# cloudflare/circl

Measured on AMD Instinct MI355X. Metric: ML-KEM-768 encapsulations/sec (whole node), batch=2^20, higher is better.
Workload: dtype i32; 1 GPU; ML-KEM-768 Encapsulate, distinct-key (one GPU-generated key per item), batch=1048576 per GPU, inputs resident in HBM (SURVEY 8d scope i; the PCIe-inclusive host-ABI rate, scope ii, is `value_host_abi`); key_pool=1048576, parallelism=batch split per device, no collectives, mode=encaps

## Files before the change

### circl_amd/csrc/api_mlkem.hip

```cpp
#include "host_compose.h"
#include "keytable.h"
#include "mlkem_kernels.h"

#include <type_traits>
#include <utility>

using namespace circl::host;
using circl::KeyIdx;

namespace {

constexpr size_t kKemWsPerItem = 129;
size_t kem_scratch_bytes() { return 256 + max_resident_blocks() * 64 * 512; }
size_t kem_small_batch() {
    static const size_t v = [] {
        const char *e = getenv("CIRCL_HIP_KEM_SMALL");
        const int lg = e ? atoi(e) : 15;
        return lg <= 0 ? size_t(0) : size_t(1) << std::min(lg, 20);
    }();
    return v;
}
size_t kem_coop_batch() {
    static const size_t v = [] {
        const char *e = getenv("CIRCL_HIP_KEM_COOP");
// ... 42 lines not shown
    switch (kem_k(param)) {
    case 2: return f(std::integral_constant<int, 2>{});
    case 3: return f(std::integral_constant<int, 3>{});
    case 4: return f(std::integral_constant<int, 4>{});
    }
    return unknown;
}
template <class F> int kem_dev_call(int param, void *stream, F &&f) {
    if (ndev() <= 0) return CIRCL_HIP_ENODEV;
    hipStream_t st = static_cast<hipStream_t>(stream);
    return kem_with_k(param, [&](auto k) -> int { return f(k, st); });
}

template <int K> struct KemTable {
    uint8_t *base;
    size_t nkeys, padded;
    KemTable(void *b, size_t nk)
        : base(static_cast<uint8_t *>(b)), nkeys(nk), padded((nk + circl::mlkem::Geom<K>::G - 1) / circl::mlkem::Geom<K>::G * circl::mlkem::Geom<K>::G) {}
    size_t rows_bytes() const { return up256(padded * K * K * 512); }
    int16_t *rows() const { return reinterpret_cast<int16_t *>(base); }
    uint8_t *h() const { return base + rows_bytes(); }
    uint8_t *status() const { return h() + up256(nkeys * 32); }
    size_t bytes() const { return rows_bytes() + up256(nkeys * 32) + up256(nkeys); }
};
size_t kem_table_bytes_any(int param, size_t nkeys) {
    return kem_with_k(param, [&](auto k) { return KemTable<k.value>(nullptr, nkeys).bytes(); }, size_t(0));
}

struct KemWs {
    uint8_t *slot0, *slot1, *slot2, *slot3, *status_slot;
    unsigned *work;
    uint8_t *scratch;
    KemWs(void *ws, size_t n) {
        slot0 = static_cast<uint8_t *>(ws);
        slot1 = slot0 + 32 * n;
        slot2 = slot0 + 64 * n;
        slot3 = slot0 + 96 * n;
        status_slot = slot0 + 128 * n;
        work = reinterpret_cast<unsigned *>(slot0 + up256(kKemWsPerItem * n));
        scratch = slot0 + up256(kKemWsPerItem * n) + 256;
    }
};


struct KemEncArgs {
    const uint8_t *ek = nullptr;
    size_t stride = 0;
    const uint8_t *m = nullptr, *r = nullptr;
    uint8_t *ct = nullptr, *ss = nullptr, *status = nullptr;
    KeyIdx kx{};
    const int16_t *key_rows = nullptr;
    const uint8_t *kbar = nullptr, *ssrej = nullptr;
};
template <int K, int MODE, int KM> void kem_encrypt(const KemWs &w, size_t n, size_t want, const KemEncArgs &a, hipStream_t st) {
    using Gm = circl::mlkem::Geom<K>;
    constexpr int lds = KM == circl::mlkem::KM_ITEM ? Gm::LDS_SCRATCH_TOTAL : Gm::LDS_SHARED_TOTAL;
    ProfScope ps(CIRCL_HIP_KERNEL_MLKEM_ENCRYPT, st);
    auto kern = circl::mlkem::mlkem_encrypt_kernel<K, MODE, 0, true, KM>;
    const unsigned eb = std::min<unsigned>((unsigned)((n + want - 1) / want), resident_blocks(kern, lds));
    hipLaunchKernelGGL(kern, dim3(eb), dim3(64), lds, st, a.ek, a.stride, a.m, a.r, a.ct, a.ss, a.status, a.kbar, a.ssrej, w.scratch, w.work, n, a.kx,
                       a.key_rows);
}

template <int K, bool R3 = false>
int encaps_dev_impl(const uint8_t *ek, const uint8_t *m, uint8_t *ct, uint8_t *ss, uint8_t *status, size_t n,
                    void *ws, size_t ws_bytes, hipStream_t st) {
    using Gm = circl::mlkem::Geom<K>;
    using namespace circl::mlkem;
    if (n == 0) return CIRCL_HIP_OK;
    if (ws_bytes < kem_ws_min(n) || !aligned<16>(ws, ek, m, ct, ss))
        return CIRCL_HIP_EWORKSPACE;
    KemWs w(ws, n);
    uint8_t *r_ws = w.slot0, *m_ws = w.slot1;
    const unsigned hb = (unsigned)((n + 255) / 256);
    if (!R3 && n <= kem_chain_item_batch()) {
        ProfScope ps(CIRCL_HIP_KERNEL_MLKEM_ENCRYPT, st);
        hipLaunchKernelGGL((mlkem_encaps_chain_kernel<K, false>), dim3((unsigned)n), dim3(128), 0, st, ek, (size_t)Gm::EK, KeyIdx{},
                           (const int16_t *)nullptr, (const uint8_t *)nullptr, m, ct, ss, status, n);
        HIP_TRY(hipGetLastError());
        return CIRCL_HIP_OK;
    }
    if (!R3 && kem_small_route(n, ws_bytes)) {
        int16_t *key_rows = reinterpret_cast<int16_t *>(static_cast<uint8_t *>(ws) + kem_small_table_ofs(n));
        const int coop = kem_hash_form(n, kem_coop_batch());
        const unsigned nb_expand = (unsigned)((n + Gm::G - 1) / Gm::G), nb_hash = kem_hash_blocks(n, coop);
        static_assert(Gm::LDS_FIFO >= 108 * 8, "the cooperative hash's exchange area fits the FIFO area");
        HIP_TRY(hipMemsetAsync(w.work, 0, 256, st));
        {
            ProfScope ps(CIRCL_HIP_KERNEL_MLKEM_HASH, st);
            hipLaunchKernelGGL(mlkem_small_pre_kernel<K>, dim3(nb_hash + nb_expand), dim3(64), Gm::LDS_FIFO, st, ek, m, ss, r_ws, key_rows, n, nb_hash, coop);
        }
        kem_encrypt<K, ENCAPS, KM_KEYED>(w, n, kem_small_group(n), {ek, (size_t)Gm::EK, m, r_ws, ct, ss, status, KeyIdx{}, key_rows}, st);
        HIP_TRY(hipGetLastError());
        return CIRCL_HIP_OK;
    }
    HIP_TRY(hipMemsetAsync(w.work, 0, 256, st));
    {
        ProfScope ps(CIRCL_HIP_KERNEL_MLKEM_HASH, st);
        if (R3) hipLaunchKernelGGL(kyber_r3_hash_kernel<K>, dim3(hb), dim3(256), 0, st, ek, m, ss, r_ws, m_ws, n);
        else hipLaunchKernelGGL(mlkem_hash_kernel<K>, dim3(hb), dim3(256), 0, st, ek, m, ss, r_ws, n);
    }
    kem_encrypt<K, R3 ? ENCAPS_LENIENT : ENCAPS, KM_ITEM>(w, n, Gm::G, {ek, (size_t)Gm::EK, R3 ? (const uint8_t *)m_ws : m, r_ws, ct, ss, status}, st);
    if (R3) {
        ProfScope ps(CIRCL_HIP_KERNEL_MLKEM_HASH, st);
        hipLaunchKernelGGL(kyber_r3_finish_kernel<K>, dim3(hb), dim3(256), 0, st, (const uint8_t *)ct, ss, n);
    }
    HIP_TRY(hipGetLastError());
    return CIRCL_HIP_OK;
}

template <int K>
int encaps_shared_dev_impl(const uint8_t *ek, const uint8_t *m, uint8_t *ct, uint8_t *ss, uint8_t *status, size_t n, void *ws,
                           size_t ws_bytes, hipStream_t st) {
    using Gm = circl::mlkem::Geom<K>;
    using namespace circl::mlkem;
    if (n == 0) return CIRCL_HIP_OK;
    if (ws_bytes < kem_ws_min(n) || !aligned<16>(ws, ek, m, ct, ss))
        return CIRCL_HIP_EWORKSPACE;
    KemWs w(ws, n);
    uint8_t *r_ws = w.slot0, *h_ws = w.slot1;
    if (n <= kem_chain_item_batch()) {
        ProfScope ps(CIRCL_HIP_KERNEL_MLKEM_ENCRYPT, st);
        hipLaunchKernelGGL((mlkem_encaps_chain_kernel<K, false>), dim3((unsigned)n), dim3(128), 0, st, ek, (size_t)0, KeyIdx{},
                           (const int16_t *)nullptr, (const uint8_t *)nullptr, m, ct, ss, status, n);
        HIP_TRY(hipGetLastError());
        return CIRCL_HIP_OK;
    }
    HIP_TRY(hipMemsetAsync(w.work, 0, 256, st));
    if (n <= kem_small_shared_batch(false)) {
        int16_t *key_rows = reinterpret_cast<int16_t *>(static_cast<uint8_t *>(ws) + kem_small_table_ofs(n));
        static_assert(Gm::LDS_FIFO >= 108 * 8, "the cooperative hash's exchange area fits the FIFO area");
        {
            ProfScope ps(CIRCL_HIP_KERNEL_MLKEM_HASH, st);
            hipLaunchKernelGGL(mlkem_small_shared_pre_kernel<K>, dim3(1 + (unsigned)((n + 31) / 32)), dim3(64), Gm::LDS_FIFO, st, ek, m, ss, r_ws, key_rows, n);
        }
        kem_encrypt<K, ENCAPS, KM_KEYED>(w, n, kem_small_group(n), {ek, 0, m, r_ws, ct, ss, status, KeyIdx{}, key_rows}, st);
        HIP_TRY(hipGetLastError());
        return CIRCL_HIP_OK;
    }
    {
        ProfScope ps(CIRCL_HIP_KERNEL_MLKEM_HASH, st);
        hipLaunchKernelGGL(mlkem_hek_kernel<K>, dim3(1), dim3(64), 0, st, ek, h_ws);
        hipLaunchKernelGGL(mlkem_g_shared_kernel, dim3((unsigned)((n + 255) / 256)), dim3(256), 0, st, (const uint8_t *)h_ws, m, ss,
                           r_ws, n, KeyIdx{});
    }
    kem_encrypt<K, ENCAPS, KM_SHARED>(w, n, Gm::GS, {ek, 0, m, r_ws, ct, ss, status}, st);
    HIP_TRY(hipGetLastError());
    return CIRCL_HIP_OK;
}

template <int K>
int decaps_shared_dev_impl(const uint8_t *dk, const uint8_t *ct, uint8_t *ss, uint8_t *status, size_t n, void *ws, size_t ws_bytes,
                           hipStream_t st) {
    using Gm = circl::mlkem::Geom<K>;
    using namespace circl::mlkem;
// ... 71 lines not shown
                               mprime, kbar, r_ws, ssrej, status, (uint8_t *)nullptr, key_rows, n, nb_hash, nb_hash, coop);
        }
        kem_encrypt<K, REENCRYPT, KM_KEYED>(w, n, kem_small_group(n, true),
                                            {dk + 384 * K, (size_t)Gm::DK, mprime, r_ws, const_cast<uint8_t *>(ct), ss, status, KeyIdx{}, key_rows, kbar, ssrej}, st);
        HIP_TRY(hipGetLastError());
        return CIRCL_HIP_OK;
    }
    {
        ProfScope ps(CIRCL_HIP_KERNEL_MLKEM_DECRYPT, st);
        hipLaunchKernelGGL(mlkem_decrypt_kernel<K>, dim3((unsigned)n), dim3(64), 0, st, dk, (size_t)Gm::DK, ct, mprime, n, KeyIdx{});
    }
    {
        ProfScope ps(CIRCL_HIP_KERNEL_MLKEM_HASH, st);
        if (R3)
            hipLaunchKernelGGL(kyber_r3_decaps_hash_kernel<K>, dim3(hb), dim3(256), 0, st, dk, (const uint8_t *)mprime, kbar, r_ws,
                               ssrej, status, n);
        else
            hipLaunchKernelGGL(mlkem_decaps_hash_kernel<K>, dim3(hb), dim3(256), 0, st, dk, (size_t)Gm::DK, ct, (const uint8_t *)mprime,
                               kbar, r_ws, ssrej, status, n, (const uint8_t *)nullptr, KeyIdx{});
    }
    kem_encrypt<K, REENCRYPT, KM_ITEM>(w, n, Gm::G,
                                       {dk + 384 * K, (size_t)Gm::DK, mprime, r_ws, const_cast<uint8_t *>(ct), ss, status, KeyIdx{}, nullptr, kbar, ssrej}, st);
    if (R3) {
        ProfScope ps(CIRCL_HIP_KERNEL_MLKEM_HASH, st);
        hipLaunchKernelGGL(kyber_r3_finish_kernel<K>, dim3(hb), dim3(256), 0, st, ct, ss, n);
    }
    HIP_TRY(hipGetLastError());
    return CIRCL_HIP_OK;
}

template <int K, bool R3 = false>
int keygen_dev_impl(const uint8_t *seed64, uint8_t *ek, uint8_t *dk, size_t n, void *ws, size_t ws_bytes, hipStream_t st) {
    using Gm = circl::mlkem::Geom<K>;
    using namespace circl::mlkem;
    if (n == 0) return CIRCL_HIP_OK;
    if (ws_bytes < kem_ws_min(n) || !aligned<16>(ws, seed64, ek, dk)) return CIRCL_HIP_EWORKSPACE;
    KemWs w(ws, n);
    uint8_t *rs = w.slot0;
    if (n <= kem_chain_item_batch()) {
        ProfScope ps(CIRCL_HIP_KERNEL_MLKEM_KEYGEN, st);
        hipLaunchKernelGGL((mlkem_keygen_chain_kernel<K, R3>), dim3((unsigned)n), dim3(128), 0, st, seed64, ek, dk, n);
        HIP_TRY(hipGetLastError());
        return CIRCL_HIP_OK;
    }
    HIP_TRY(hipMemsetAsync(w.work, 0, 256, st));
    const unsigned hb = (unsigned)((n + 255) / 256);
    {
        ProfScope ps(CIRCL_HIP_KERNEL_MLKEM_HASH, st);
        hipLaunchKernelGGL((mlkem_keygen_seed_kernel<K, R3>), dim3(hb), dim3(256), 0, st, seed64, rs, n);
    }
    {
        ProfScope ps(CIRCL_HIP_KERNEL_MLKEM_KEYGEN, st);
        auto kern = mlkem_keygen_kernel<K, true>;
        const unsigned kb = std::min<unsigned>((unsigned)((n + Gm::G - 1) / Gm::G), resident_blocks(kern, Gm::LDS_SCRATCH_TOTAL));
        hipLaunchKernelGGL(kern, dim3(kb), dim3(64), Gm::LDS_SCRATCH_TOTAL, st, (const uint8_t *)rs, ek, dk, w.scratch, w.work, n);
    }
    {
        ProfScope ps(CIRCL_HIP_KERNEL_MLKEM_FINISH, st);
        const int form = n <= (size_t(1) << 15) ? kem_hash_form(n, kem_coop_batch()) : 0;
        if (form) hipLaunchKernelGGL(mlkem_keygen_finish_small_kernel<K>, dim3(kem_hash_blocks(n, form)), dim3(64), 0, st, seed64, (const uint8_t *)ek, dk, n, form);
        else hipLaunchKernelGGL(mlkem_keygen_finish_kernel<K>, dim3(hb), dim3(256), 0, st, seed64, (const uint8_t *)ek, dk, n);
    }
    HIP_TRY(hipGetLastError());
    return CIRCL_HIP_OK;
}


template <int K> void kem_table_fill(const KemTable<K> &tb, const uint8_t *keys, size_t row, bool private_keys, hipStream_t st) {
    using Gm = circl::mlkem::Geom<K>;
    using namespace circl::mlkem;
    const size_t ek_off = private_keys ? 384 * K : 0, rho_off = ek_off + 384 * K;
    hipLaunchKernelGGL(mlkem_hek_table_kernel<K>, dim3((unsigned)((tb.nkeys + 255) / 256)), dim3(256), 0, st, keys, row, ek_off, tb.h(),
                       private_keys ? tb.status() : (uint8_t *)nullptr, private_keys ? 1 : 0, tb.nkeys);
    hipLaunchKernelGGL(mlkem_expand_keys_kernel<K>, dim3((unsigned)(tb.padded / Gm::G)), dim3(64), Gm::LDS_FIFO, st, keys, row, rho_off, tb.rows(), tb.nkeys);
}

template <int K>
int encaps_with_table(const KemTable<K> &tb, const uint8_t *keys, size_t stride, KeyIdx kx, bool latency, const uint8_t *m, uint8_t *ct, uint8_t *ss,
                      uint8_t *status, size_t n, const KemWs &w, hipStream_t st) {
    using Gm = circl::mlkem::Geom<K>;
    using namespace circl::mlkem;
    uint8_t *r_ws = w.slot0;
    if (latency && n <= kem_chain_batch(false)) {
        ProfScope ps(CIRCL_HIP_KERNEL_MLKEM_ENCRYPT, st);
        circl::TailFlag tail{nullptr, nullptr, 0};
        take_tail_flag(&tail.flag, &tail.count, &tail.value);
        hipLaunchKernelGGL(mlkem_encaps_chain_kernel<K>, dim3((unsigned)n), dim3(64), 0, st, keys, (size_t)Gm::EK, kx, (const int16_t *)tb.rows(),
                           (const uint8_t *)tb.h(), m, ct, ss, status, n, tail);
        HIP_TRY(hipGetLastError());
        return CIRCL_HIP_OK;
    }
    HIP_TRY(hipMemsetAsync(w.work, 0, 256, st));
    {
        ProfScope ps(CIRCL_HIP_KERNEL_MLKEM_HASH, st);
        hipLaunchKernelGGL(mlkem_g_shared_kernel, dim3((unsigned)((n + 255) / 256)), dim3(256), 0, st, (const uint8_t *)tb.h(), m, ss, r_ws, n, kx);
    }
    const size_t want = latency && n <= kem_small_shared_batch(false) ? kem_small_group(n) : (size_t)Gm::GS;
    kem_encrypt<K, ENCAPS, KM_KEYED>(w, n, want, {keys, stride, m, r_ws, ct, ss, status, kx, tb.rows()}, st);
    HIP_TRY(hipGetLastError());
    return CIRCL_HIP_OK;
}
template <int K>
int decaps_with_table(const KemTable<K> &tb, const uint8_t *dk, size_t stride, KeyIdx kx, bool latency, const uint8_t *ct, uint8_t *ss, uint8_t *status,
                      size_t n, const KemWs &w, hipStream_t st) {
    using Gm = circl::mlkem::Geom<K>;
    using namespace circl::mlkem;
    uint8_t *mprime = w.slot0, *r_ws = w.slot1, *kbar = w.slot2, *ssrej = w.slot3;
// ... 446 lines not shown
```

### circl_amd/csrc/mlkem_kernels.h

```cpp
#pragma once
#include "kyber_dev.h"

#ifndef CIRCL_KEM_RING_PRIO
#define CIRCL_KEM_RING_PRIO 1
#endif
#ifndef CIRCL_KEM_WAVES_PER_EU
#define CIRCL_KEM_WAVES_PER_EU 4
#endif

namespace circl {
namespace mlkem {

using kyber::Q;

template <int K> struct Params;
template <> struct Params<2> { static constexpr int ETA1 = 3, DU = 10, DV = 4; };
template <> struct Params<3> { static constexpr int ETA1 = 2, DU = 10, DV = 4; };
template <> struct Params<4> { static constexpr int ETA1 = 2, DU = 11, DV = 5; };

template <int K> struct Geom {
    using P = Params<K>;
    static constexpr int EK = 384 * K + 32;
    static constexpr int DK = 768 * K + 96;
    static constexpr int CT = 32 * (P::DU * K + P::DV);
    static constexpr int PAIRS = K * K;
    static constexpr int G = 64 / PAIRS;
    static constexpr int A_STREAMS = G * PAIRS;
    static constexpr int NOISE = 2 * K + 1;
    static constexpr int A_STRIDE = 520;
    static constexpr int NOISE_BYTES = 64 * P::ETA1;
    static constexpr int NOISE_STRIDE = NOISE_BYTES + 8;
    static constexpr int LDS_A = A_STREAMS * A_STRIDE;
    static constexpr int HALVES = K == 2 ? 2 : 1;
    static constexpr int GH = G / HALVES;
    static constexpr int LDS_NOISE = GH * NOISE * NOISE_STRIDE;
    static constexpr int LDS_XCH = 1024;
    static constexpr int LDS_TOTAL = LDS_A + LDS_NOISE + LDS_XCH;
    static constexpr int FIFO_STRIDE = 80;
    static constexpr int LDS_FIFO = 64 * FIFO_STRIDE;
    static constexpr int LDS_SCRATCH_TOTAL = (LDS_FIFO > LDS_NOISE + LDS_XCH) ? LDS_FIFO : LDS_NOISE + LDS_XCH;
    static constexpr int SCRATCH_BYTES = 64 * 512;
    static constexpr int GS = K == 2 ? 8 : 64 / NOISE;
    static constexpr int LDS_NOISE_SHARED = GS * NOISE * NOISE_STRIDE;
    static constexpr int LDS_SHARED_TOTAL = (LDS_FIFO > LDS_NOISE_SHARED + LDS_XCH) ? LDS_FIFO : LDS_NOISE_SHARED + LDS_XCH;
};


template <int FIRST, int COUNT> __device__ __forceinline__ void xor_words(KeccakState &s, const uint64_t *p) {
    detail::static_for<0, COUNT>([&](auto ic) {
        constexpr int i = decltype(ic)::v;
        const uint64_t w = p[i];
        s.lo[FIRST + i] ^= (uint32_t)w;
        s.hi[FIRST + i] ^= (uint32_t)(w >> 32);
    });
}

template <int NWORDS> __device__ __forceinline__ void sha3_256_words(KeccakState &s, const uint64_t *p) {
    constexpr int FULL = NWORDS / 17, REM = NWORDS % 17;
    keccak_zero(s);
#pragma unroll 1
    for (int b = 0; b < FULL; b++) {
        xor_words<0, 17>(s, p + 17 * b);
        keccak_f1600(s);
    }
    xor_words<0, REM>(s, p + 17 * FULL);
    s.lo[REM] ^= kDsSha3;
    s.hi[16] ^= 0x80000000u;
    keccak_f1600(s);
}

__device__ __forceinline__ void sha3_512_m_h(KeccakState &g, const uint64_t *m, const KeccakState &h) {
    keccak_zero(g);
    xor_words<0, 4>(g, m);
#pragma unroll
    for (int i = 0; i < 4; i++) { g.lo[4 + i] = h.lo[i]; g.hi[4 + i] = h.hi[i]; }
    g.lo[8] = kDsSha3;
    g.hi[8] = 0x80000000u;
    keccak_f1600(g);
}

template <int NWORDS, class Src> __device__ __forceinline__ void split_sponge17_src(SplitState &s, Src &&src, uint32_t ds, bool hi_lane) {
    constexpr int FULL = NWORDS / 17, REM = NWORDS % 17;
    uint32_t nx[17];
#pragma unroll
    for (int j = 0; j < 25; j++) s.w[j] = 0;
#pragma unroll
    for (int j = 0; j < 17; j++) nx[j] = (FULL > 0 || j < REM) ? src(j) : 0;
#pragma unroll 1
    for (int b = 0; b < FULL; b++) {
#pragma unroll
        for (int j = 0; j < 17; j++) s.w[j] ^= nx[j];
        const bool last = b + 1 == FULL;
#pragma unroll
// ... 15 lines not shown
    const uint32_t *mw = reinterpret_cast<const uint32_t *>(m + item * 32) + parity;
    SplitState s;
#pragma unroll
    for (int j = 0; j < 4; j++) { s.w[j] = mw[2 * j]; s.w[4 + j] = h[j]; }
    s.w[8] = hi_lane ? 0x80000000u : kDsSha3;
#pragma unroll
    for (int j = 9; j < 25; j++) s.w[j] = 0;
    keccak_f1600_split(s, hi_lane);
    if (live) {
        uint32_t *kd = reinterpret_cast<uint32_t *>(ss + item * 32) + parity, *rd = reinterpret_cast<uint32_t *>(r_ws + item * 32) + parity;
#pragma unroll
        for (int j = 0; j < 4; j++) { kd[2 * j] = s.w[j]; rd[2 * j] = s.w[4 + j]; }
    }
}
template <int K>
__device__ __forceinline__ void mlkem_hash_split(const uint8_t *__restrict__ ek, const uint8_t *__restrict__ m, uint8_t *__restrict__ ss,
                                                 uint8_t *__restrict__ r_ws, size_t item, bool live, int parity) {
    using Gm = Geom<K>;
    SplitState s;
    split_sponge17<Gm::EK / 8>(s, reinterpret_cast<const uint32_t *>(ek + item * Gm::EK) + parity, kDsSha3, parity != 0);
    const uint32_t h[4] = {s.w[0], s.w[1], s.w[2], s.w[3]};
    mlkem_g_split(h, m, ss, r_ws, item, live, parity);
}

template <int FIRST, int COUNT> __device__ __forceinline__ void store_words(uint64_t *p, const KeccakState &s) {
    detail::static_for<0, COUNT>([&](auto ic) {
        constexpr int i = decltype(ic)::v;
        p[i] = ((uint64_t)s.hi[FIRST + i] << 32) | s.lo[FIRST + i];
    });
}

template <bool NW = false, class Src>
__device__ __forceinline__ void coop_sponge17(uint32_t &vlo, uint32_t &vhi, Src &&src, int nwords, uint32_t ds, const CoopLane &c, int j) {
    const int full = nwords / 17, rem = nwords % 17;
    vlo = vhi = 0;
    uint64_t next = j < 17 ? src(j) : 0;
#pragma unroll 1
    for (int b = 0; b < full; b++) {
        vlo ^= (uint32_t)next;
        vhi ^= (uint32_t)(next >> 32);
        next = (j < 17 && 17 * (b + 1) + j < nwords) ? src(17 * (b + 1) + j) : 0;
        keccak_f1600_coop2<NW>(vlo, vhi, c);
    }
    vlo ^= (uint32_t)next;
    vhi ^= (uint32_t)(next >> 32);
    if (j == rem) vlo ^= ds;
    if (j == 16) vhi ^= 0x80000000u;
    keccak_f1600_coop2<NW>(vlo, vhi, c);
}


template <int K>
__global__ void __launch_bounds__(256) mlkem_hash_kernel(const uint8_t *__restrict__ ek, const uint8_t *__restrict__ m,
                                                         uint8_t *__restrict__ ss, uint8_t *__restrict__ r_ws, size_t n) {
    using Gm = Geom<K>;
    size_t idx = (size_t)blockIdx.x * 256 + threadIdx.x;
    const bool live = idx < n;
    if (!live) idx = n - 1;
    KeccakState h, g;
    sha3_256_words<Gm::EK / 8>(h, reinterpret_cast<const uint64_t *>(ek + idx * Gm::EK));
    sha3_512_m_h(g, reinterpret_cast<const uint64_t *>(m + idx * 32), h);
    if (live) {
        store_words<0, 4>(reinterpret_cast<uint64_t *>(ss + idx * 32), g);
        store_words<4, 4>(reinterpret_cast<uint64_t *>(r_ws + idx * 32), g);
    }
}

template <int K>
__global__ void __launch_bounds__(64) mlkem_dk_check_kernel(const uint8_t *__restrict__ dk, uint8_t *__restrict__ key_status) {
    __shared__ uint64_t ws[100];
    const int lane = threadIdx.x, j = lane & 31;
    const CoopLane c = coop_lane(ws, lane);
    const uint64_t *ekw = reinterpret_cast<const uint64_t *>(dk + 384 * K);
    const uint64_t *stored = reinterpret_cast<const uint64_t *>(dk + 768 * K + 32);
    uint32_t vlo, vhi;
    coop_sponge17(vlo, vhi, [&](int k) { return ekw[k]; }, Geom<K>::EK / 8, kDsSha3, c, j);
    const bool mine = j >= 4 || ((((uint64_t)vhi << 32) | vlo) == stored[j & 3]);
    const unsigned long long bad = __ballot(!mine);
    if (lane == 0) *key_status = (bad & 0xfull) == 0 ? 0 : 2;
}


template <int K>
__global__ void __launch_bounds__(64) mlkem_hek_kernel(const uint8_t *__restrict__ ek, uint8_t *__restrict__ h_ws) {
    __shared__ uint64_t ws[100];
    const int lane = threadIdx.x, j = lane & 31;
    const CoopLane c = coop_lane(ws, lane);
    const uint64_t *ekw = reinterpret_cast<const uint64_t *>(ek);
    uint32_t vlo, vhi;
    coop_sponge17(vlo, vhi, [&](int k) { return ekw[k]; }, Geom<K>::EK / 8, kDsSha3, c, j);
    if (lane < 4) reinterpret_cast<uint64_t *>(h_ws)[lane] = ((uint64_t)vhi << 32) | vlo;
}

template <int K>
__global__ void __launch_bounds__(256) mlkem_hek_table_kernel(const uint8_t *__restrict__ keys, size_t stride, size_t ek_off,
                                                              uint8_t *__restrict__ h_out, uint8_t *__restrict__ key_status, int stored,
                                                              size_t nkeys) {
    size_t j = (size_t)blockIdx.x * 256 + threadIdx.x;
    const bool live = j < nkeys;
    if (!live) j = nkeys - 1;
    const uint8_t *ekp = keys + j * stride + ek_off;
    KeccakState h;
    sha3_256_words<Geom<K>::EK / 8>(h, reinterpret_cast<const uint64_t *>(ekp));
    if (!live) return;
    store_words<0, 4>(reinterpret_cast<uint64_t *>(h_out + j * 32), h);
    if (stored) {
        const uint64_t *st = reinterpret_cast<const uint64_t *>(ekp + Geom<K>::EK);
        bool ok = true;
#pragma unroll
        for (int i = 0; i < 4; i++) ok &= (((uint64_t)h.hi[i] << 32) | h.lo[i]) == st[i];
        key_status[j] = ok ? 0 : 2;
    }
}
// ... 142 lines not shown
            fifo[cnt & (SLOTS - 1)] = (int16_t)v;
            count_accept(cnt, v);
            if constexpr (c % 8 == 7) {
                cnt = min(cnt, 256);
                if (cnt - flushed >= 8) {
                    const uint4 d = *reinterpret_cast<const uint4 *>(fifo + (flushed & (SLOTS - 1)));
                    *reinterpret_cast<uint4 *>(row + flushed) = d;
                    flushed += 8;
                }
                if constexpr (TAIL) live = __any(flushed < 256);
            }
        }
    });
}

template <int K, bool TRANSPOSED, int GA = Geom<K>::G, bool XY_ARG = false>
__device__ __forceinline__ void sample_matrix_scratch(uint8_t *lds_fifo, int16_t *rows, const uint8_t *__restrict__ rho,
                                                      size_t rho_stride, size_t item0, size_t n, int lane, const uint8_t *__restrict__ xy = nullptr) {
    using Gm = Geom<K>;
    const bool on = XY_ARG ? item0 + lane < n : lane < GA * Gm::PAIRS;
    const int g = XY_ARG ? lane : on ? lane / Gm::PAIRS : 0, p = on ? lane % Gm::PAIRS : 0;
    const int i = p / K, j = p % K;
    size_t item = item0 + g;
    if (item >= n) item = n - 1;
    KeccakState s;
    keccak_zero(s);
    xor_words<0, 4>(s, reinterpret_cast<const uint64_t *>(rho + item * rho_stride));
    if constexpr (XY_ARG) s.lo[4] = (uint32_t)xy[2 * item] | ((uint32_t)xy[2 * item + 1] << 8) | (kDsShake << 16);
    else s.lo[4] = (TRANSPOSED ? (uint32_t)i | ((uint32_t)j << 8) : (uint32_t)j | ((uint32_t)i << 8)) | (kDsShake << 16);
    s.hi[20] = 0x80000000u;
    int16_t *fifo = reinterpret_cast<int16_t *>(lds_fifo + lane * Gm::FIFO_STRIDE);
    int16_t *row = rows + lane * 256;
    int cnt = on ? 0 : 256, flushed = cnt;
#pragma unroll 1
    for (int blk = 0; blk < 3; blk++) {
        keccak_f1600(s);
        if (on) parse_shake128_block_fifo<false>(s, fifo, row, cnt, flushed);
    }
#pragma unroll 1
    while (__any(flushed < 256)) {
        keccak_f1600(s);
        parse_shake128_block_fifo<true>(s, fifo, row, cnt, flushed);
    }
}

template <bool ETA2> __device__ __forceinline__ void store_prf_words(uint32_t *out, const KeccakState &s) {
    detail::static_for<0, 16>([&](auto ic) {
        constexpr int w = decltype(ic)::v;
        out[2 * w] = ETA2 ? kyber::cbd2_bias8_word(s.lo[w]) : s.lo[w];
        out[2 * w + 1] = ETA2 ? kyber::cbd2_bias8_word(s.hi[w]) : s.hi[w];
    });
}

template <int K, bool TRANSPOSED, int NOISE, int ETA1_COUNT>
__device__ __forceinline__ void sample_matrix_and_prf(uint8_t *lds_fifo, uint8_t *lds_noise, uint8_t *lds_mini, int16_t *rows,
                                                      const uint8_t *__restrict__ rho, size_t rho_stride,
                                                      const uint8_t *__restrict__ seed, size_t seed_stride, size_t item0, size_t n,
                                                      int lane) {
    using Gm = Geom<K>;
    constexpr int STREAMS = Gm::G * NOISE;
    constexpr int LAST_BASE = ((STREAMS - 1) / 64) * 64, USED_LAST = STREAMS - LAST_BASE, FREE = 64 - USED_LAST;
    constexpr int MAX_HITCH = FREE < 15 ? FREE : 15;
    constexpr bool CAN_HITCH = Params<K>::ETA1 == 2 && MAX_HITCH > 0;
    constexpr int STASH = 240;
    static_assert(15 * STASH <= Gm::LDS_FIFO, "stash fits in the FIFO area");

    KeccakState s;
    int cnt, flushed;
    int16_t *fifo = reinterpret_cast<int16_t *>(lds_fifo + lane * Gm::FIFO_STRIDE);
    {
        const bool on = lane < Gm::A_STREAMS;
        const int g = on ? lane / Gm::PAIRS : 0, p = on ? lane % Gm::PAIRS : 0;
        const int i = p / K, j = p % K;
        size_t item = item0 + g;
        if (item >= n) item = n - 1;
        keccak_zero(s);
        xor_words<0, 4>(s, reinterpret_cast<const uint64_t *>(rho + item * rho_stride));
        s.lo[4] = (TRANSPOSED ? (uint32_t)i | ((uint32_t)j << 8) : (uint32_t)j | ((uint32_t)i << 8)) | (kDsShake << 16);
        s.hi[20] = 0x80000000u;
        int16_t *row = rows + lane * 256;
        cnt = on ? 0 : 256;
        flushed = cnt;
#pragma unroll 1
        for (int blk = 0; blk < 3; blk++) {
            keccak_f1600(s);
            if (on) parse_shake128_block_fifo<false>(s, fifo, row, cnt, flushed);
        }
        const unsigned long long smask0 = __ballot(flushed < 256);
        if (!CAN_HITCH || __popcll(smask0) > MAX_HITCH) {
#pragma unroll 1
            while (__any(flushed < 256)) {
                keccak_f1600(s);
                parse_shake128_block_fifo<true>(s, fifo, row, cnt, flushed);
            }
        }
    }
    const unsigned long long smask = __ballot(flushed < 256);
    const int nstr = __popcll(smask);
    if (nstr > 0) {
        const bool mine = (smask >> lane) & 1;
        uint4 pend = make_uint4(0, 0, 0, 0);
        if (mine) pend = *reinterpret_cast<const uint4 *>(fifo + (flushed & 31));
        __syncthreads();
        if (mine) {
            uint32_t *st = reinterpret_cast<uint32_t *>(lds_fifo + __popcll(smask & ((1ull << lane) - 1)) * STASH);
#pragma unroll
            for (int w = 0; w < 25; w++) { st[2 * w] = s.lo[w]; st[2 * w + 1] = s.hi[w]; }
            st[50] = (uint32_t)cnt; st[51] = (uint32_t)flushed; st[52] = (uint32_t)lane;
            st[53] = pend.x; st[54] = pend.y; st[55] = pend.z; st[56] = pend.w;
        }
    }
    __syncthreads();

#pragma unroll 1
    for (int base = 0; base < STREAMS; base += 64) {
        const int sidx = base + lane;
        const bool on = sidx < STREAMS;
        const int g = on ? sidx / NOISE : 0, nonce = on ? sidx % NOISE : 0;
        size_t item = item0 + g;
        if (item >= n) item = n - 1;
        keccak_zero(s);
        xor_words<0, 4>(s, reinterpret_cast<const uint64_t *>(seed + item * seed_stride));
        s.lo[4] = (uint32_t)nonce | (kDsShake << 8);
        s.hi[16] = 0x80000000u;
        const bool adopt_pass = CAN_HITCH && nstr > 0 && base == LAST_BASE;
        const int tk = lane - USED_LAST;
        const bool target = adopt_pass && tk >= 0 && tk < nstr;
        int tcnt = 256, tflushed = 256, tsrc = 0;
        uint4 pend = make_uint4(0, 0, 0, 0);
        if (target) {
            const uint32_t *st = reinterpret_cast<const uint32_t *>(lds_fifo + tk * STASH);
#pragma unroll
            for (int w = 0; w < 25; w++) { s.lo[w] = st[2 * w]; s.hi[w] = st[2 * w + 1]; }
            tcnt = (int)st[50]; tflushed = (int)st[51]; tsrc = (int)st[52];
            pend = make_uint4(st[53], st[54], st[55], st[56]);
        }
        keccak_f1600(s);
        uint32_t *out = reinterpret_cast<uint32_t *>(lds_noise + (on ? sidx : 0) * Gm::NOISE_STRIDE);
        if constexpr (Params<K>::ETA1 == 2) {
            if (on) store_prf_words<true>(out, s);
        } else {
            if (on && nonce < ETA1_COUNT) store_prf_words<false>(out, s);
            if (on && nonce >= ETA1_COUNT) store_prf_words<true>(out, s);
        }
        if constexpr (Params<K>::ETA1 == 3) {
            if (on && nonce < ETA1_COUNT) { out[32] = s.lo[16]; out[33] = s.hi[16]; }
            if (__any(on && nonce < ETA1_COUNT)) {
                keccak_f1600(s);
                if (on && nonce < ETA1_COUNT) {
                    detail::static_for<0, 7>([&](auto ic) {
                        constexpr int w = decltype(ic)::v;
                        out[34 + 2 * w] = s.lo[w];
                        out[35 + 2 * w] = s.hi[w];
                    });
                }
            }
        }
        if (adopt_pass) {
            int16_t *tf = reinterpret_cast<int16_t *>(lds_mini + (target ? tk : 15) * 32);
            int16_t *trow = rows + tsrc * 256;
            if (target) *reinterpret_cast<uint4 *>(tf + (tflushed & 15)) = pend;
            parse_shake128_block_fifo<true, 16>(s, tf, trow, tcnt, tflushed);
#pragma unroll 1
            while (__any(tflushed < 256)) {
                keccak_f1600(s);
                parse_shake128_block_fifo<true, 16>(s, tf, trow, tcnt, tflushed);
            }
        }
    }
}

struct AFromLds {
    const uint8_t *base;
    int stride;
    __device__ __forceinline__ void load(uint32_t &a01, uint32_t &a23, int stream, int lane) const {
        const uint2 w = *reinterpret_cast<const uint2 *>(base + stream * stride + 8 * lane);
        a01 = w.x; a23 = w.y;
    }
};
struct AFromScratch {
    const int16_t *rows;
    __device__ __forceinline__ void load(uint32_t &a01, uint32_t &a23, int stream, int lane) const {
        const uint64_t w = __hip_atomic_load(reinterpret_cast<const uint64_t *>(rows + stream * 256 + 4 * lane), __ATOMIC_RELAXED,
                                             __HIP_MEMORY_SCOPE_AGENT);
        a01 = (uint32_t)w; a23 = (uint32_t)(w >> 32);
    }
};
struct AFromCache {
    const int16_t *rows;
    __device__ __forceinline__ void load(uint32_t &a01, uint32_t &a23, int stream, int lane) const {
// ... 211 lines not shown
    if (sh + D > 16) w |= (unsigned)p[b + 2] << 16;
    return (w >> sh) & ((1u << D) - 1);
}

__device__ __forceinline__ size_t next_group(unsigned *work, int lane, bool first, size_t ngroups) {
    if (first) return (size_t)blockIdx.x;
    if (work == nullptr || (size_t)gridDim.x >= ngroups) return ngroups;
    unsigned t = 0;
    if (lane == 0) t = atomicAdd(work, 1u);
    return (size_t)gridDim.x + (size_t)(unsigned)__builtin_amdgcn_readfirstlane((int)t);
}


enum EncryptMode { ENCAPS = 0, REENCRYPT = 1, ENCAPS_LENIENT = 2 };

enum KeyMode { KM_ITEM = 0, KM_SHARED = 1, KM_KEYED = 2 };
template <int K, int MODE, int ABLATE_ARG = 0, bool SCRATCH = true, int KM = KM_ITEM>
__global__ void __launch_bounds__(64, SCRATCH ? CIRCL_KEM_WAVES_PER_EU : 1) mlkem_encrypt_kernel(const uint8_t *__restrict__ ek, size_t ek_stride,
                                                          const uint8_t *__restrict__ m, const uint8_t *__restrict__ r_ws,
                                                          uint8_t *__restrict__ ct, uint8_t *__restrict__ ss,
                                                          uint8_t *__restrict__ status, const uint8_t *__restrict__ kbar_ws,
                                                          const uint8_t *__restrict__ ssrej_ws, uint8_t *__restrict__ scratch, unsigned *__restrict__ work, size_t n,
                                                          const KeyIdx key_idx, const int16_t *__restrict__ key_rows) {
    using Gm = Geom<K>;
    using P = Params<K>;
    constexpr int ABLATE = ABLATE_ARG & 7;
    constexpr bool CLK = (ABLATE_ARG & 8) != 0;
    uint64_t clk[4] = {0, 0, 0, 0}, tprev = 0;
    auto lap = [&](int slot) {
        if constexpr (CLK) {
            const uint64_t t = __builtin_readcyclecounter();
            clk[slot] += t - tprev;
            tprev = t;
        }
    };
    if constexpr (CLK) tprev = __builtin_readcyclecounter();
    extern __shared__ __attribute__((aligned(16))) uint8_t smem[];
    uint8_t *lds_a = smem;
    uint8_t *lds_noise = SCRATCH ? smem : smem + Gm::LDS_A;
    constexpr bool SHARED = KM != KM_ITEM;
    static_assert(!SHARED || (SCRATCH && (MODE == ENCAPS || MODE == REENCRYPT) && ABLATE == 0), "shared-key / key-table mode");
    uint8_t *xch = lds_noise + (SHARED ? Gm::LDS_NOISE_SHARED : Gm::LDS_NOISE);
    int16_t *rows = KM == KM_KEYED ? nullptr : reinterpret_cast<int16_t *>(scratch + (size_t)blockIdx.x * Gm::SCRATCH_BYTES);
    const int lane = threadIdx.x;
    constexpr int GI = SHARED ? Gm::GS : Gm::G;
    const unsigned gi = (SHARED && (size_t)gridDim.x * GI >= n) ? (unsigned)((n + gridDim.x - 1) / gridDim.x) : (unsigned)GI;
    const size_t ngroups = (n + gi - 1) / gi;
    if constexpr (KM == KM_SHARED) {
        sample_matrix_scratch<K, true, 1>(lds_a, rows, ek + 384 * K, 0, 0, 1, lane);
        __threadfence_block();
        __syncthreads();
    }

#pragma unroll 1
  for (size_t grp = next_group(work, lane, true, ngroups); grp < ngroups; grp = next_group(work, lane, false, ngroups)) {
    const size_t item0 = grp * gi;
    lap(0);
    if constexpr (CIRCL_KEM_RING_PRIO != 0) __builtin_amdgcn_s_setprio(0);
    if constexpr (SHARED) {
        __syncthreads();
        if (gi * Gm::NOISE <= 32) prf_streams_split<K, Gm::NOISE, K>(lds_noise, r_ws, 32, item0, n, lane, (int)gi);
        else prf_streams<K, Gm::NOISE, K, Gm::GS>(lds_noise, r_ws, 32, item0, n, lane);
        __syncthreads();
    } else if constexpr (SCRATCH && ABLATE == 0 && Gm::HALVES == 1) {
        __syncthreads();
        sample_matrix_and_prf<K, true, Gm::NOISE, K>(lds_a, lds_noise, xch, rows, ek + 384 * K, ek_stride,
                                                     r_ws, 32, item0, n, lane);
        __threadfence_block();
        __syncthreads();
    } else {
        if (!(ABLATE & 1)) {
            if constexpr (SCRATCH) {
                __syncthreads();
                sample_matrix_scratch<K, true>(lds_a, rows, ek + 384 * K, ek_stride, item0, n, lane);
                __threadfence_block();
            } else {
                sample_matrix<K, true>(lds_a, ek + 384 * K, ek_stride, item0, n, lane);
            }
        }
        __syncthreads();
        if constexpr (Gm::HALVES == 1) {
            if (!(ABLATE & 2)) prf_streams<K, Gm::NOISE, K>(lds_noise, r_ws, 32, item0, n, lane);
            __syncthreads();
        }
    }

    int lane_ring = lane;
    asm volatile("" : "+v"(lane_ring));
    if constexpr (CIRCL_KEM_RING_PRIO != 0) __builtin_amdgcn_s_setprio(CIRCL_KEM_RING_PRIO);
    lap(1);
    const kyber::LaneZetas z = kyber::load_lane_zetas(lane_ring);
#pragma unroll 1
    for (int g = 0; g < ((ABLATE & 4) ? 0 : (int)gi); g++) {
        const size_t item = item0 + g;
        if (item >= n) break;
        if constexpr (Gm::HALVES > 1 && !SHARED) {
            if (g % Gm::GH == 0) {
                __syncthreads();
                if (!(ABLATE & 2)) prf_streams<K, Gm::NOISE, K, Gm::GH>(lds_noise, r_ws, 32, item0, n, lane, g);
                __syncthreads();
            }
        }
        const size_t kq = KM == KM_KEYED ? (key_idx ? (size_t)key_idx[item] : (ek_stride ? item : size_t(0))) : item;
        const uint8_t *ekp = ek + kq * ek_stride;
        const int16_t *krows = KM == KM_KEYED ? key_rows + kq * (size_t)(K * K * 256) : nullptr;
        const uint8_t *noise = lds_noise + (SHARED ? g : g % Gm::GH) * Gm::NOISE * Gm::NOISE_STRIDE;

        int th[K][4];
        bool bad = false;
#pragma unroll
        for (int j = 0; j < K; j++) {
            unpack12_l4(th[j], ekp + 384 * j, lane);
// ... 32 lines not shown
                else AFromLds{lds_a, Gm::A_STRIDE}.load(a01, a23, (g * K + i) * K + j, lane);
                kyber::mulhat_acc_packed(acc, a01, a23, rop[j]);
            }
            kyber::mulhat_finish(acc);
            kyber::invntt<kyber::NEG_R32, CIRCL_KEM_RING_XCH>(acc, z, xch, lane);
            const uint8_t *e1 = noise + (K + i) * Gm::NOISE_STRIDE;
            unsigned cv[4];
#pragma unroll
            for (int r = 0; r < 4; r++)
                cv[r] = kyber::compress_coeff<P::DU>(acc[r] + cbd_coeff<2>(e1, kyber::idx_l1(lane, r)));
            uint32_t *stage = reinterpret_cast<uint32_t *>(xch);
            stage_bits_l1<P::DU>(stage, cv, lane);
            if (MODE == REENCRYPT) differs |= ref.differs(stage, lane);
            else store_staged<P::DU>(dst, stage, lane, reject);
        }
        {
            uint32_t *dst = reinterpret_cast<uint32_t *>(ctp + 32 * P::DU * K);
            RefWords<P::DV> ref;
            if (MODE == REENCRYPT) ref.load(dst, lane);
            int acc[4] = {0, 0, 0, 0};
#pragma unroll
            for (int j = 0; j < K; j++) kyber::mulhat_acc_packed(acc, kyber::pack16(th[j][0], th[j][1]), kyber::pack16(th[j][2], th[j][3]), rop[j]);
            kyber::mulhat_finish(acc);
            kyber::invntt<kyber::NEG_R32, CIRCL_KEM_RING_XCH>(acc, z, xch, lane);
            const uint8_t *e2 = noise + 2 * K * Gm::NOISE_STRIDE;
            const uint8_t *mp = m + item * 32;
            unsigned cv[4];
#pragma unroll
            for (int r = 0; r < 4; r++) {
                const int nidx = kyber::idx_l1(lane, r);
                const int mbit = (mp[nidx >> 3] >> (nidx & 7)) & 1;
                cv[r] = kyber::compress_coeff<P::DV>(acc[r] + cbd_coeff<2>(e2, nidx) + (-mbit & ((Q + 1) / 2)));
            }
            uint32_t *stage = reinterpret_cast<uint32_t *>(xch);
            stage_bits_l1<P::DV>(stage, cv, lane);
            if (MODE == REENCRYPT) differs |= ref.differs(stage, lane);
            else store_staged<P::DV>(dst, stage, lane, reject);
        }
        if (MODE == ENCAPS) {
            if (lane == 0) status[item] = reject ? 1 : 0;
            if (reject && lane < 8) reinterpret_cast<uint32_t *>(ss + item * 32)[lane] = 0;
        } else if (MODE == REENCRYPT) {
            const bool mismatch = __any(differs);
            const bool dead = status[item] != 0;
            if (lane < 8) {
                const uint32_t kb = reinterpret_cast<const uint32_t *>(kbar_ws + item * 32)[lane];
                const uint32_t rj = reinterpret_cast<const uint32_t *>(ssrej_ws + item * 32)[lane];
                reinterpret_cast<uint32_t *>(ss + item * 32)[lane] = dead ? 0u : (mismatch ? rj : kb);
            }
        }
        if constexpr (CLK) clk[3]++;
    }
    lap(2);
  }
    if constexpr (CLK) {
        lap(0);
        if (lane == 0) {
            uint64_t *prof = reinterpret_cast<uint64_t *>(const_cast<int16_t *>(key_rows)) + (size_t)blockIdx.x * 4;
#pragma unroll
            for (int q = 0; q < 4; q++) prof[q] = clk[q];
        }
    }
}

template <int K>
__global__ void __launch_bounds__(64, CIRCL_KEM_WAVES_PER_EU) mlkem_expand_keys_kernel(const uint8_t *__restrict__ keys, size_t stride, size_t rho_off,
                                                                                      int16_t *__restrict__ key_rows, size_t nkeys) {
    using Gm = Geom<K>;
    extern __shared__ __attribute__((aligned(16))) uint8_t smem[];
    const size_t e0 = (size_t)blockIdx.x * Gm::G;
    sample_matrix_scratch<K, true>(smem, key_rows + e0 * (size_t)(K * K * 256), keys + rho_off, stride, e0, nkeys, threadIdx.x);
}

template <int K>
__device__ __forceinline__ void mlkem_hash_coop2(const uint8_t *__restrict__ ek, const uint8_t *__restrict__ m, uint8_t *__restrict__ ss,
                                                 uint8_t *__restrict__ r_ws, size_t item0, size_t n, uint64_t *ws, int lane) {
    using Gm = Geom<K>;
    constexpr int NW = Gm::EK / 8, FULL = NW / 17, REM = NW % 17;
    const CoopLane c = coop_lane(ws, lane);
    uint64_t *hx = ws + 100;
    const int half = lane >> 5, j = lane & 31;
    size_t item = item0 + half;
    const bool live = item < n;
    if (!live) item = n - 1;
    const uint64_t *ekw = reinterpret_cast<const uint64_t *>(ek + item * Gm::EK);
    uint32_t vlo = 0, vhi = 0;
    uint64_t next = j < 17 ? ekw[j] : 0;
#pragma unroll 1
    for (int b = 0; b < FULL; b++) {
        vlo ^= (uint32_t)next;
        vhi ^= (uint32_t)(next >> 32);
        next = (j < 17 && 17 * (b + 1) + j < NW) ? ekw[17 * (b + 1) + j] : 0;
        keccak_f1600_coop2(vlo, vhi, c);
    }
    vlo ^= (uint32_t)next;
    vhi ^= (uint32_t)(next >> 32);
    if (j == REM) vlo ^= kDsSha3;
    if (j == 16) vhi ^= 0x80000000u;
    keccak_f1600_coop2(vlo, vhi, c);
    __syncthreads();
    if (j < 4) hx[4 * half + j] = ((uint64_t)vhi << 32) | vlo;
    __syncthreads();
    uint64_t g = 0;
    if (j < 4) g = reinterpret_cast<const uint64_t *>(m + item * 32)[j];
    else if (j < 8) g = hx[4 * half + j - 4];
    else if (j == 8) g = 0x8000000000000000ull | kDsSha3;
// ... 908 lines not shown
```

Baseline: 146.8 million encaps/s.

## Fold G-hash of next group into idle PRF lanes of encrypt kernel

```diff
diff --git a/circl_amd/csrc/api_mlkem.hip b/circl_amd/csrc/api_mlkem.hip
--- a/circl_amd/csrc/api_mlkem.hip
+++ b/circl_amd/csrc/api_mlkem.hip
@@ -118,12 +118,26 @@
     const int16_t *key_rows = nullptr;
     const uint8_t *kbar = nullptr, *ssrej = nullptr;
 };
+unsigned kem_max_wgs() {
+    static const int v = env_int("CIRCL_HIP_KEM_MAX_WGS", 0, 1, 1 << 30);
+    return v > 0 ? (unsigned)v : ~0u;
+}
+template <int K, int MODE, int KM> constexpr bool kem_g_rides() {
+    return CIRCL_KEM_G_RIDE != 0 && KM == circl::mlkem::KM_ITEM && MODE == circl::mlkem::ENCAPS && circl::mlkem::Geom<K>::HALVES == 1;
+}
+template <int K, int MODE, int KM> constexpr int kem_encrypt_lds() {
+    using Gm = circl::mlkem::Geom<K>;
+    return KM != circl::mlkem::KM_ITEM ? Gm::LDS_SHARED_TOTAL : kem_g_rides<K, MODE, KM>() ? Gm::LDS_GRIDE_TOTAL : Gm::LDS_SCRATCH_TOTAL;
+}
+template <int K, int MODE, int KM> unsigned kem_encrypt_grid(size_t n, size_t want) {
+    auto kern = circl::mlkem::mlkem_encrypt_kernel<K, MODE, 0, true, KM>;
+    return std::min({(unsigned)((n + want - 1) / want), resident_blocks(kern, kem_encrypt_lds<K, MODE, KM>()), kem_max_wgs()});
+}
 template <int K, int MODE, int KM> void kem_encrypt(const KemWs &w, size_t n, size_t want, const KemEncArgs &a, hipStream_t st) {
-    using Gm = circl::mlkem::Geom<K>;
-    constexpr int lds = KM == circl::mlkem::KM_ITEM ? Gm::LDS_SCRATCH_TOTAL : Gm::LDS_SHARED_TOTAL;
+    constexpr int lds = kem_encrypt_lds<K, MODE, KM>();
     ProfScope ps(CIRCL_HIP_KERNEL_MLKEM_ENCRYPT, st);
     auto kern = circl::mlkem::mlkem_encrypt_kernel<K, MODE, 0, true, KM>;
-    const unsigned eb = std::min<unsigned>((unsigned)((n + want - 1) / want), resident_blocks(kern, lds));
+    const unsigned eb = kem_encrypt_grid<K, MODE, KM>(n, want);
     hipLaunchKernelGGL(kern, dim3(eb), dim3(64), lds, st, a.ek, a.stride, a.m, a.r, a.ct, a.ss, a.status, a.kbar, a.ssrej, w.scratch, w.work, n, a.kx,
                        a.key_rows);
 }
@@ -161,12 +175,20 @@
         return CIRCL_HIP_OK;
     }
     HIP_TRY(hipMemsetAsync(w.work, 0, 256, st));
+    constexpr int MODE = R3 ? ENCAPS_LENIENT : ENCAPS;
+    constexpr bool ride = kem_g_rides<K, MODE, KM_ITEM>();
+    uint8_t *h_ws = ride ? w.slot1 : nullptr;
+    static_assert(kKemWsPerItem >= 64, "r and H(ek): two 32-byte slots per item");
     {
         ProfScope ps(CIRCL_HIP_KERNEL_MLKEM_HASH, st);
         if (R3) hipLaunchKernelGGL(kyber_r3_hash_kernel<K>, dim3(hb), dim3(256), 0, st, ek, m, ss, r_ws, m_ws, n);
-        else hipLaunchKernelGGL(mlkem_hash_kernel<K>, dim3(hb), dim3(256), 0, st, ek, m, ss, r_ws, n);
-    }
-    kem_encrypt<K, R3 ? ENCAPS_LENIENT : ENCAPS, KM_ITEM>(w, n, Gm::G, {ek, (size_t)Gm::EK, R3 ? (const uint8_t *)m_ws : m, r_ws, ct, ss, status}, st);
+        else {
+            size_t g_items = n;
+            if (ride) g_items = (std::min(n, (size_t)kem_encrypt_grid<K, MODE, KM_ITEM>(n, Gm::G) * Gm::G) + 255) / 256 * 256;
+            hipLaunchKernelGGL(mlkem_hash_kernel<K>, dim3(hb), dim3(256), 0, st, ek, m, ss, r_ws, n, h_ws, g_items);
+        }
+    }
+    kem_encrypt<K, MODE, KM_ITEM>(w, n, Gm::G, {ek, (size_t)Gm::EK, R3 ? (const uint8_t *)m_ws : m, r_ws, ct, ss, status, KeyIdx{}, nullptr, h_ws}, st);
     if (R3) {
         ProfScope ps(CIRCL_HIP_KERNEL_MLKEM_HASH, st);
         hipLaunchKernelGGL(kyber_r3_finish_kernel<K>, dim3(hb), dim3(256), 0, st, (const uint8_t *)ct, ss, n);
@@ -344,7 +366,7 @@
     {
         ProfScope ps(CIRCL_HIP_KERNEL_MLKEM_KEYGEN, st);
         auto kern = mlkem_keygen_kernel<K, true>;
-        const unsigned kb = std::min<unsigned>((unsigned)((n + Gm::G - 1) / Gm::G), resident_blocks(kern, Gm::LDS_SCRATCH_TOTAL));
+        const unsigned kb = std::min({(unsigned)((n + Gm::G - 1) / Gm::G), resident_blocks(kern, Gm::LDS_SCRATCH_TOTAL), kem_max_wgs()});
         hipLaunchKernelGGL(kern, dim3(kb), dim3(64), Gm::LDS_SCRATCH_TOTAL, st, (const uint8_t *)rs, ek, dk, w.scratch, w.work, n);
     }
     {
diff --git a/circl_amd/csrc/mlkem_kernels.h b/circl_amd/csrc/mlkem_kernels.h
--- a/circl_amd/csrc/mlkem_kernels.h
+++ b/circl_amd/csrc/mlkem_kernels.h
@@ -3,6 +3,9 @@
 
 #ifndef CIRCL_KEM_RING_PRIO
 #define CIRCL_KEM_RING_PRIO 1
+#endif
+#ifndef CIRCL_KEM_G_RIDE
+#define CIRCL_KEM_G_RIDE 1
 #endif
 #ifndef CIRCL_KEM_WAVES_PER_EU
 #define CIRCL_KEM_WAVES_PER_EU 4
@@ -39,6 +42,8 @@
     static constexpr int FIFO_STRIDE = 80;
     static constexpr int LDS_FIFO = 64 * FIFO_STRIDE;
     static constexpr int LDS_SCRATCH_TOTAL = (LDS_FIFO > LDS_NOISE + LDS_XCH) ? LDS_FIFO : LDS_NOISE + LDS_XCH;
+    static constexpr int LDS_GRIDE_TOTAL = LDS_SCRATCH_TOTAL + 256 + 512;
+    static_assert(G * 32 <= 256 || K == 2, "the r stash of a group fits");
     static constexpr int SCRATCH_BYTES = 64 * 512;
     static constexpr int GS = K == 2 ? 8 : 64 / NOISE;
     static constexpr int LDS_NOISE_SHARED = GS * NOISE * NOISE_STRIDE;
@@ -160,13 +165,16 @@
 
 template <int K>
 __global__ void __launch_bounds__(256) mlkem_hash_kernel(const uint8_t *__restrict__ ek, const uint8_t *__restrict__ m,
-                                                         uint8_t *__restrict__ ss, uint8_t *__restrict__ r_ws, size_t n) {
+                                                         uint8_t *__restrict__ ss, uint8_t *__restrict__ r_ws, size_t n,
+                                                         uint8_t *__restrict__ h_ws = nullptr, size_t g_items = ~size_t(0)) {
     using Gm = Geom<K>;
     size_t idx = (size_t)blockIdx.x * 256 + threadIdx.x;
     const bool live = idx < n;
     if (!live) idx = n - 1;
     KeccakState h, g;
     sha3_256_words<Gm::EK / 8>(h, reinterpret_cast<const uint64_t *>(ek + idx * Gm::EK));
+    if (h_ws != nullptr && live) store_words<0, 4>(reinterpret_cast<uint64_t *>(h_ws + idx * 32), h);
+    if ((size_t)blockIdx.x * 256 >= g_items) return;
     sha3_512_m_h(g, reinterpret_cast<const uint64_t *>(m + idx * 32), h);
     if (live) {
         store_words<0, 4>(reinterpret_cast<uint64_t *>(ss + idx * 32), g);
@@ -415,19 +423,31 @@
     });
 }
 
-template <int K, bool TRANSPOSED, int NOISE, int ETA1_COUNT>
+struct GRide {
+    bool on = false;
+    size_t item0 = 0;
+    const uint8_t *m = nullptr, *h = nullptr;
+    uint8_t *ss = nullptr, *r = nullptr, *mh = nullptr;
+};
+struct GRideNone {
+    __device__ __forceinline__ GRide operator()() const { return GRide{}; }
+};
+template <int K, bool TRANSPOSED, int NOISE, int ETA1_COUNT, bool GRIDE = false, class RideFn = GRideNone>
 __device__ __forceinline__ void sample_matrix_and_prf(uint8_t *lds_fifo, uint8_t *lds_noise, uint8_t *lds_mini, int16_t *rows,
                                                       const uint8_t *__restrict__ rho, size_t rho_stride,
                                                       const uint8_t *__restrict__ seed, size_t seed_stride, size_t item0, size_t n,
-                                                      int lane) {
+                                                      int lane, RideFn &&ride_fn = RideFn{}) {
     using Gm = Geom<K>;
     constexpr int STREAMS = Gm::G * NOISE;
     constexpr int LAST_BASE = ((STREAMS - 1) / 64) * 64, USED_LAST = STREAMS - LAST_BASE, FREE = 64 - USED_LAST;
-    constexpr int MAX_HITCH = FREE < 15 ? FREE : 15;
+    constexpr int GLANES = GRIDE ? Gm::G : 0;
+    static_assert(!GRIDE || (FREE >= Gm::G && Params<K>::ETA1 == 2), "the G lanes fit the idle lanes of a one-permutation PRF pass");
+    constexpr int MAX_HITCH = FREE - GLANES < 15 ? FREE - GLANES : 15;
     constexpr bool CAN_HITCH = Params<K>::ETA1 == 2 && MAX_HITCH > 0;
     constexpr int STASH = 240;
     static_assert(15 * STASH <= Gm::LDS_FIFO, "stash fits in the FIFO area");
 
+    GRide ride;
     KeccakState s;
     int cnt, flushed;
     int16_t *fifo = reinterpret_cast<int16_t *>(lds_fifo + lane * Gm::FIFO_STRIDE);
@@ -439,6 +459,20 @@
         if (item >= n) item = n - 1;
         keccak_zero(s);
         xor_words<0, 4>(s, reinterpret_cast<const uint64_t *>(rho + item * rho_stride));
+        if constexpr (GRIDE) {
+            ride = ride_fn();
+            int lane_g = lane;
+            asm volatile("" : "+v"(lane_g));
+            if (ride.on && lane_g < GLANES * 4) {
+                size_t gi = ride.item0 + (lane_g >> 2);
+                if (gi >= n) gi = n - 1;
+                const uint64_t mw = reinterpret_cast<const uint64_t *>(ride.m + gi * 32)[lane_g & 3];
+                const uint64_t hw = reinterpret_cast<const uint64_t *>(ride.h + gi * 32)[lane_g & 3];
+                uint64_t *dst = reinterpret_cast<uint64_t *>(ride.mh + (lane_g >> 2) * 64) + (lane_g & 3);
+                dst[0] = mw;
+                dst[4] = hw;
+            }
+        }
         s.lo[4] = (TRANSPOSED ? (uint32_t)i | ((uint32_t)j << 8) : (uint32_t)j | ((uint32_t)i << 8)) | (kDsShake << 16);
         s.hi[20] = 0x80000000u;
         int16_t *row = rows + lane * 256;
@@ -482,12 +516,29 @@
         const int g = on ? sidx / NOISE : 0, nonce = on ? sidx % NOISE : 0;
         size_t item = item0 + g;
         if (item >= n) item = n - 1;
+        int lane_g = lane;
+        if constexpr (GRIDE) asm volatile("" : "+v"(lane_g));
+        const int gk = lane_g - USED_LAST;
+        bool glane = false;
+        if constexpr (GRIDE) glane = ride.on && base == LAST_BASE && gk >= 0 && gk < GLANES;
         keccak_zero(s);
-        xor_words<0, 4>(s, reinterpret_cast<const uint64_t *>(seed + item * seed_stride));
-        s.lo[4] = (uint32_t)nonce | (kDsShake << 8);
-        s.hi[16] = 0x80000000u;
+        if constexpr (GRIDE) {
+            if (glane) {
+                xor_words<0, 8>(s, reinterpret_cast<const uint64_t *>(ride.mh + gk * 64));
+                s.lo[8] = kDsSha3;
+                s.hi[8] = 0x80000000u;
+            } else {
+                xor_words<0, 4>(s, reinterpret_cast<const uint64_t *>(ride.r + g * 32));
+                s.lo[4] = (uint32_t)nonce | (kDsShake << 8);
+                s.hi[16] = 0x80000000u;
+            }
+        } else {
+            xor_words<0, 4>(s, reinterpret_cast<const uint64_t *>(seed + item * seed_stride));
+            s.lo[4] = (uint32_t)nonce | (kDsShake << 8);
+            s.hi[16] = 0x80000000u;
+        }
         const bool adopt_pass = CAN_HITCH && nstr > 0 && base == LAST_BASE;
-        const int tk = lane - USED_LAST;
+        const int tk = lane - USED_LAST - GLANES;
         const bool target = adopt_pass && tk >= 0 && tk < nstr;
         int tcnt = 256, tflushed = 256, tsrc = 0;
         uint4 pend = make_uint4(0, 0, 0, 0);
@@ -499,6 +550,13 @@
             pend = make_uint4(st[53], st[54], st[55], st[56]);
         }
         keccak_f1600(s);
+        if constexpr (GRIDE) {
+            if (glane) {
+                const size_t gi = ride.item0 + gk;
+                if (gi < n) store_words<0, 4>(reinterpret_cast<uint64_t *>(ride.ss + gi * 32), s);
+                store_words<4, 4>(reinterpret_cast<uint64_t *>(ride.r + gk * 32), s);
+            }
+        }
         uint32_t *out = reinterpret_cast<uint32_t *>(lds_noise + (on ? sidx : 0) * Gm::NOISE_STRIDE);
         if constexpr (Params<K>::ETA1 == 2) {
             if (on) store_prf_words<true>(out, s);
@@ -816,12 +874,32 @@
         __syncthreads();
     }
 
-#pragma unroll 1
-  for (size_t grp = next_group(work, lane, true, ngroups); grp < ngroups; grp = next_group(work, lane, false, ngroups)) {
+    constexpr bool GRIDE = CIRCL_KEM_G_RIDE != 0 && KM == KM_ITEM && MODE == ENCAPS && SCRATCH && ABLATE_ARG == 0 && Gm::HALVES == 1;
+    uint8_t *r_stash = smem + Gm::LDS_SCRATCH_TOTAL;
+    if constexpr (GRIDE) {
+        if (lane < Gm::G * 8) {
+            size_t item = (size_t)blockIdx.x * Gm::G + (lane >> 3);
+            if (item >= n) item = n - 1;
+            reinterpret_cast<uint32_t *>(r_stash)[lane] = reinterpret_cast<const uint32_t *>(r_ws + item * 32)[lane & 7];
+        }
+    }
+
+#pragma unroll 1
+  for (size_t grp = next_group(work, lane, true, ngroups); grp < ngroups;) {
     const size_t item0 = grp * gi;
+    size_t grp_next = ngroups;
     lap(0);
     if constexpr (CIRCL_KEM_RING_PRIO != 0) __builtin_amdgcn_s_setprio(0);
-    if constexpr (SHARED) {
+    if constexpr (GRIDE) {
+        __syncthreads();
+        auto draw = [&]() {
+            grp_next = next_group(work, lane, false, ngroups);
+            return GRide{grp_next < ngroups, grp_next * Gm::G, m, kbar_ws, ss, r_stash, r_stash + 256};
+        };
+        sample_matrix_and_prf<K, true, Gm::NOISE, K, true>(lds_a, lds_noise, xch, rows, ek + 384 * K, ek_stride, nullptr, 0, item0, n, lane, draw);
+        __threadfence_block();
+        __syncthreads();
+    } else if constexpr (SHARED) {
         __syncthreads();
         if (gi * Gm::NOISE <= 32) prf_streams_split<K, Gm::NOISE, K>(lds_noise, r_ws, 32, item0, n, lane, (int)gi);
         else prf_streams<K, Gm::NOISE, K, Gm::GS>(lds_noise, r_ws, 32, item0, n, lane);
@@ -960,6 +1038,8 @@
         if constexpr (CLK) clk[3]++;
     }
     lap(2);
+    if constexpr (GRIDE) grp = grp_next;
+    else grp = next_group(work, lane, false, ngroups);
   }
     if constexpr (CLK) {
         lap(0);
```

New measurement: 146.9 million encaps/s, median of 5. No clear change (+0.1%).
